# PrivEimantas/myFYP

Hardware: AMD Instinct MI355X
Metric: rounds/sec + wall-clock-to-target-acc, MNIST MLP FedAvg 8 peers at 1/2/4/8 MI355X (higher is better)
Workload: dtype fp32

## Files before the change

csrc/kernels/mlp_persistent.h:

```cpp
#pragma once
#include "mlp_fused.h"

struct MLPPersistBufs {
  bf16* h1x;
  bf16* w2x;
  bf16* dh2x;
  unsigned* flags;
  size_t flag_bytes;
  int* err;
  int plain_ok;
  int plain;
};

bool mlp_persistent_supported(const MLPArgs& a);
size_t mlp_persistent_bytes(int P, int Bpad);
size_t mlp_persistent_flag_bytes(int P);
int mlp_persistent_blocks(int P);
hipError_t mlp_persistent_prepare(const MLPArgs& a);
hipError_t mlp_launch_persistent_epoch(const MLPArgs& a, const MLPPersistBufs& pb, hipStream_t s, bool zero_flags = true);

struct MLPPersistF32Bufs {
  float* h1x;
  float* plx;
  float* dh2x;
  unsigned* gen;
  unsigned* flags;
  size_t flag_bytes;
  int* err;
  unsigned fbase;
  float* w2chk;
  int plain_ok;
  int plain;
  int plain_x;
  int c2_straight;
};

int mlp_plain_pub_mode();
bool mlp_persistent_f32_supported(const MLPArgs& a);
size_t mlp_persistent_f32_h1x_floats(int P, int Bpad);
size_t mlp_persistent_f32_bytes(int P, int Bpad);
size_t mlp_persistent_f32_flag_bytes(int P);
int mlp_persistent_f32_gang();
int mlp_persistent_f32_resident_capacity(const MLPArgs& a, int num_cus);
int mlp_persistent_f32_launch_wgs(const MLPArgs& a);
int mlp_persistent_f32_ks(const MLPArgs& a);
int mlp_persistent_f32_variant(const MLPArgs& a);
int mlp_persistent_f32_flags_per_peer();
void mlp_persistent_f32_flag_layout(int* line, int* lines_per_peer, int* full_lines);
hipError_t mlp_persistent_f32_prepare(const MLPArgs& a);
hipError_t mlp_launch_persistent_f32_epoch(const MLPArgs& a, const MLPPersistF32Bufs& pb, hipStream_t s, bool zero_flags = true,
                                           const int* active = nullptr);
void mlp_launch_eval_f32(const MLPArgs& a, int max_rows, hipStream_t s);
```

csrc/kernels/mlp_persistent_f32.hip:

```cpp
#include <atomic>

#include "mlp_persistent.h"
#include "persist_common.h"
#include "mlp_f32_common.h"

bool mlp_f32v2_supported(const MLPArgs& a);
size_t mlp_f32v2_lds(const MLPArgs& a);
size_t mlp_f32v2_bytes(int P, int Bpad);
int mlp_f32v2_launch_wgs();
int mlp_f32v2_resident_capacity(const MLPArgs& a, int num_cus);
hipError_t mlp_f32v2_prepare(const MLPArgs& a);
void mlp_f32v2_launch(const MLPArgs& a, const MLPPersistF32Bufs& pb, hipStream_t s);

#ifdef MLP_STAMPS
__device__ unsigned long long g_p32_stamps[2][128][10];
__device__ unsigned long long g_p32_epoch[4];
#define P32_STAMP(role, t, i)                                                                    \
  do {                                                                                           \
    if (p == 0 && threadIdx.x == 0 && (t) < 128) g_p32_stamps[role][t][i] = wall_clock64(); \
  } while (0)
#define P32_ESTAMP(i)                                        \
  do {                                                       \
    if (p == 0 && threadIdx.x == 0) g_p32_epoch[i] = wall_clock64(); \
  } while (0)
#define P32_STAMP_W1(t, i)                                                                   \
  do {                                                                                       \
    if (p == 0 && threadIdx.x == 64 && (t) < 128) g_p32_stamps[0][t][i] = wall_clock64(); \
  } while (0)
extern "C" int mlp_debug_persistent_f32_stamps(void* out) {
  return hipMemcpyFromSymbol(out, HIP_SYMBOL(g_p32_stamps), sizeof(g_p32_stamps)) == hipSuccess ? 0 : 1;
}
extern "C" int mlp_debug_persistent_f32_epoch_stamps(void* out) {
  return hipMemcpyFromSymbol(out, HIP_SYMBOL(g_p32_epoch), sizeof(g_p32_epoch)) == hipSuccess ? 0 : 1;
}
#else
#define P32_STAMP(role, t, i) \
  do {                        \
  } while (0)
#define P32_ESTAMP(i) \
  do {                \
  } while (0)
#define P32_STAMP_W1(t, i) \
  do {                     \
  } while (0)
#endif

__device__ int g_plain_seen[64];

namespace {

using persist::al16;
using persist::gu32;
using persist::row_max16;
using persist::row_min16;
using persist::row_sum16;
using namespace f32k;

constexpr int SMR = 2;
constexpr int LDT_PAD = 16;
constexpr int NCG = 16;
constexpr int NH = 8;
constexpr int KSMAX = 8;
constexpr int KSLAB = KSMAX + 1;
__host__ __device__ constexpr int ng_of(int KS) { return NCG * KS; }
__host__ __device__ constexpr int roles_of(int KS) { return NCG * KS + NH; }
__host__ __device__ constexpr bool xr_of(int KS, bool RH) { return KS > 1 && !RH; }
__host__ __device__ constexpr int ppl_of(int KS, bool RH = false) { return RH ? (KS == 1 ? 8 : 4) : 8 / KS; }
__host__ __device__ constexpr int grid_of(int KS, bool RH, int nr) { return RH ? ppl_of(KS, true) * nr : 8 * (NCG + NH); }
__host__ __device__ inline int kpart_begin(int ks1, int KS, int kh) { return (kh * ks1) / KS; }
constexpr int F_H1 = 0;
constexpr int F_H1P = NCG;
constexpr int F_PL = NCG + NCG * KSMAX, F_DH2 = F_PL + NH, F_DONE = F_DH2 + NH;
constexpr int FPP = F32_FPP;
constexpr int F_XCC = F32_FPP - 5;
static_assert(F_DONE + NCG * KSMAX + NH <= F_XCC, "layout-1 flags fit the shared block");
static_assert(roles_of(KSMAX) <= 5 * 32, "XCC report slots");
constexpr int F3_DH2 = NCG * KSMAX;
constexpr int F3_W2 = F3_DH2 + 4;
constexpr int F3_HP = F3_W2 + NCG;
constexpr int F3_DONE = F3_HP + 4;
static_assert(F3_DONE + NCG * KSMAX + 4 <= F_XCC, "layout-3 flags fit the shared block");
__host__ __device__ constexpr int nhr_of(int BP) { return BP / 16; }
__host__ __device__ constexpr int roles3_of(int KS, int BP) { return NCG * KS + nhr_of(BP); }
constexpr int HPW = 16 * PD2 + PD2 + 16;
__host__ __device__ inline size_t v3_extra_floats(int P) { return (size_t)P * PD2 * PD1 + (size_t)P * 2 * 4 * HPW; }
constexpr int KS1_MAX = 25;


__device__ __forceinline__ float* h1x_part(const MLPPersistF32Bufs& pb, int p, int kh, int t, int BP) {
  return pb.h1x + (((int64_t)p * KSLAB + kh) * 2 + (t & 1)) * BP * PD1;
}
__device__ __forceinline__ float* h1x_red(const MLPPersistF32Bufs& pb, int p, int t, int BP) { return h1x_part(pb, p, KSMAX, t, BP); }


__device__ __forceinline__ bf16x8 frag_b_tr_x(const bf16* base, int ld, int k0, int s, int tt, int lane) {
  const int g = lane >> 4, q = (lane & 15) >> 2, pp = lane & 3;
  const int cx = 2 * tt + (pp >> 1);
  const bf16* p0 = base + (k0 + 8 * g + q) * ld + 32 * s + (cx << 3) + 4 * (pp & 1);
  const bf16* p1 = p0 + 4 * ld;
  const mlp_s16x4 lo = __builtin_amdgcn_ds_read_tr16_b64_v4i16((mlp_lds_s16x4*)(p0));
  const mlp_s16x4 hi = __builtin_amdgcn_ds_read_tr16_b64_v4i16((mlp_lds_s16x4*)(p1));
  return __builtin_bit_cast(bf16x8, (mlp_s16x8)__builtin_shufflevector(lo, hi, 0, 1, 2, 3, 4, 5, 6, 7));
}

struct OwnerLds32 {
  int ldx;
  int ldt;
  size_t x, red, h1, dh1s, w1x, ok, total;
};
__host__ __device__ inline int kh_of(int D0, int KS) { return (ks1_of(D0) + KS - 1) / KS; }
__host__ __device__ inline OwnerLds32 owner_lds32(int Bpad, int D0, int KS) {
  OwnerLds32 L;
  L.ldx = kh_of(D0, KS) * 32 + 8;
  L.ldt = Bpad + LDT_PAD;
  const int MT = Bpad / 16;
  const size_t red = (size_t)8 * MT * 64 * 16, dh2 = (size_t)Bpad * LDD * 4;
  size_t o = 0;
  L.x = o;    o += al16((size_t)Bpad * L.ldx * 2);
  L.red = o;  o += al16(red > dh2 ? red : dh2);
  L.h1 = o;   o += al16((size_t)2 * Bpad * 16 * 4);
  L.dh1s = o; o += al16((size_t)3 * 16 * L.ldt * 2);
  L.w1x = o;  o += al16(KS == 1 ? (size_t)4 * 16 * 32 * 4 : 0);
  L.ok = o;   o += 16;
  L.total = o;
  return L;
}
struct HeadLds32 {
  size_t h1, red, h2, lg, dlog, dh2, w3, b2, b3, ok, total;
};
__host__ __device__ inline HeadLds32 head_lds32(int Bpad) {
  HeadLds32 L;
  const int MT = Bpad / 16;
  size_t o = 0;
  L.h1 = o;   o += al16((size_t)Bpad * LDH1 * 4);
  L.red = o;  o += al16((size_t)8 * MT * 64 * 16);
  L.h2 = o;   o += al16((size_t)Bpad * LD16 * 4);
  L.lg = o;   o += al16((size_t)Bpad * LD16 * 4);
  L.dlog = o; o += al16((size_t)Bpad * LD16 * 4);
  L.dh2 = o;  o += al16((size_t)Bpad * LD16 * 4);
  L.w3 = o;   o += al16((size_t)16 * LD16 * 4);
  L.b2 = o;   o += al16(4 * 16 * 4);
  L.b3 = o;   o += al16(4 * 16 * 4);
  L.ok = o;   o += 16;
  L.total = o;
  return L;
}

__host__ __device__ constexpr int rq_of(int KS) { return KS == 1 ? 3 : KS == 2 ? 2 : 1; }

template <int KS, bool RH = false, int BP = 64>
__device__ __forceinline__ bool gang_commit(const MLPArgs& a, const MLPPersistF32Bufs& pb, int p, int role, int* sOk) {
  if (pb.fbase == 0 && role == 0 && a.debug_giveup == p + 1 + 256) {
    if (threadIdx.x == 0) __hip_atomic_store(pb.err, 1, __ATOMIC_RELAXED, __HIP_MEMORY_SCOPE_AGENT);
    return false;
  }
  constexpr int FD = RH ? F3_DONE : F_DONE;
  constexpr int NR = RH ? roles3_of(KS, BP) : roles_of(KS);
  persist::publish(pb.flags, FPP, p, FD + role, pb.fbase + DONE_MARK);
  return persist::wg_wait(pb.flags, FPP, p, FD, NR, pb.fbase + DONE_MARK, pb.err, sOk);
}

template <int BP, bool ADAM, bool EXTRA, int KS, bool RH, bool FUSE = false>
__device__ void owner32(const MLPArgs& a, const MLPPersistF32Bufs& pb, int p, int g, char* smem) {
  static_assert(!FUSE || (KS == 1 && !RH && !EXTRA), "fused forward: layout 1, K split 1, no extra term");
  constexpr int MT = BP / 16;
  constexpr int RQ = rq_of(KS);
  constexpr int XPT = BP / 4;
  const int tid = threadIdx.x, lane = tid & 63;
  const int wave = __builtin_amdgcn_readfirstlane(tid >> 6);
  const int h = lane >> 4, c = lane & 15;
  const int cg = g % NCG, kh = g / NCG;
  const int D0 = a.D0;
  constexpr bool XR = xr_of(KS, RH);
  const int s0 = kpart_begin(ks1_of(D0), KS, kh);
  const int KS1 = kpart_begin(ks1_of(D0), KS, kh + 1) - s0;
  const int C0 = 32 * s0;
  const OwnerLds32 L = owner_lds32(BP, D0, KS);
  const int LDX = L.ldx, LDT = L.ldt;
  bf16* sX = reinterpret_cast<bf16*>(smem + L.x);
  f32x4* sRed = reinterpret_cast<f32x4*>(smem + L.red);
  float* sDH2 = reinterpret_cast<float*>(smem + L.red);
  float* sH1 = reinterpret_cast<float*>(smem + L.h1);
  bf16* sD3 = reinterpret_cast<bf16*>(smem + L.dh1s);
  float* sW1x = reinterpret_cast<float*>(smem + L.w1x);
  int* sOk = reinterpret_cast<int*>(smem + L.ok);
  const OptParams& o = a.opt;
  const int4 ctl = a.ctl[p];
  const bool fresh = (ctl.x & 2) != 0;
  const int n = ctl.y;
  const int nsteps = (n + a.B - 1) / a.B;
  const int64_t pS = (int64_t)p * a.S;
  const float wdmu = o.weight_decay + (a.anchor != nullptr ? o.mu : 0.f);

  float w1[RQ][8], m1[RQ][8], v1[RQ][8], e1[RQ][8];
  const int orow = NCG * cg + c;
#pragma unroll
  for (int q = 0; q < RQ + 1; ++q) {
    const int s = wave + 8 * q;
    if (q == RQ && (KS != 1 || s >= KS1)) break;
#pragma unroll
    for (int half = 0; half < 2; ++half) {
      const int k = C0 + 32 * s + 16 * half + 4 * h;
      float4 wv = {0.f, 0.f, 0.f, 0.f}, mv = wv, vv = wv, ev = wv;
      if (s < KS1 && k < D0) {
        const int64_t idx = pS + a.off_w1 + (int64_t)orow * D0 + k;
        wv = *reinterpret_cast<const float4*>(a.params + idx);
        if (!fresh) {
          mv = *reinterpret_cast<const float4*>(a.m + idx);
          if (ADAM) vv = *reinterpret_cast<const float4*>(a.v + idx);
        }
        if (EXTRA) ev = float4{extra_at(a, idx), extra_at(a, idx + 1), extra_at(a, idx + 2), extra_at(a, idx + 3)};
      } else if (s < KS1 && k == D0) {
        const int64_t idx = pS + a.off_b1 + orow;
        wv.x = a.params[idx];
        if (!fresh) {
          mv.x = a.m[idx];
          if (ADAM) vv.x = a.v[idx];
        }
        if (EXTRA) ev.x = extra_at(a, idx);
      }
      if (q < RQ) {
        const float wa[4] = {wv.x, wv.y, wv.z, wv.w}, ma[4] = {mv.x, mv.y, mv.z, mv.w}, va[4] = {vv.x, vv.y, vv.z, vv.w},
                    ea[4] = {ev.x, ev.y, ev.z, ev.w};
#pragma unroll
        for (int i = 0; i < 4; ++i) {
          w1[q][4 * half + i] = wa[i];
          m1[q][4 * half + i] = ma[i];
          v1[q][4 * half + i] = va[i];
          e1[q][4 * half + i] = ea[i];
        }
      } else {
        const int off = c * 32 + 16 * half + 4 * h;
        *reinterpret_cast<float4*>(sW1x + off) = wv;
        *reinterpret_cast<float4*>(sW1x + 512 + off) = mv;
        *reinterpret_cast<float4*>(sW1x + 1024 + off) = vv;
        *reinterpret_cast<float4*>(sW1x + 1536 + off) = ev;
      }
    }
  }
  float w2c[4], m2c[4], v2c[4], e2c[4];
#pragma unroll
  for (int i = 0; i < 4; ++i) {
    const int64_t idx = pS + a.off_w2 + (int64_t)(16 * wave + 4 * h + i) * PD1 + NCG * cg + c;
    w2c[i] = a.params[idx];
    m2c[i] = fresh ? 0.f : a.m[idx];
    v2c[i] = (ADAM && !fresh) ? a.v[idx] : 0.f;
    e2c[i] = EXTRA ? extra_at(a, idx) : 0.f;
  }

  auto bias_chunk = [](bool valid) { return uint4{valid ? 0x3F80u : 0u, 0u, 0u, 0u}; };
  auto xw_stage = [&](int t, int lv) {
    const int rows = rows_at(a, n, t);
#pragma unroll
    for (int k = 0; k < XPT; ++k) {
      const int q = k / (BP / 16), kk = k % (BP / 16);
      if (q > RQ || (q == RQ && KS != 1)) break;
      const int s = wave + 8 * q;
      const int idx = kk * 64 + lv;
      const int r = idx >> 2, col = 32 * s + 8 * (idx & 3), gcol = C0 + col;
      if (s < KS1 && gcol < D0) {
        const bf16* src = a.Xb16 + ((int64_t)p * a.xb_rows + (int64_t)t * a.B + r) * D0 + gcol;
        *reinterpret_cast<uint4*>(sX + r * LDX + col) = r < rows ? *reinterpret_cast<const uint4*>(src) : uint4{0u, 0u, 0u, 0u};
      } else if (s < KS1 && gcol == D0) {
        *reinterpret_cast<uint4*>(sX + r * LDX + col) = bias_chunk(r < rows);
      }
    }
  };
  {
// ... 36 lines not shown
      bf16x8 af[MT];
#pragma unroll
      for (int mt = 0; mt < MT; ++mt) {
        const bf16* xp = sX + (16 * mt + cq) * LDX + 32 * s + 4 * (hq & 1);
        af[mt] = cat8(*reinterpret_cast<const bf16x4*>(xp + ((hq >> 1) << 3)), *reinterpret_cast<const bf16x4*>(xp + ((2 + (hq >> 1)) << 3)));
      }
#pragma unroll
      for (int mt = 0; mt < MT; ++mt) acc[mt] = mfma_bf16(af[mt], bl, acc[mt]);
#pragma unroll
      for (int mt = 0; mt < MT; ++mt) acc[mt] = mfma_bf16(af[mt], bm, acc[mt]);
#pragma unroll
      for (int mt = 0; mt < MT; ++mt) acc[mt] = mfma_bf16(af[mt], bh, acc[mt]);
      return;
    }
#pragma unroll
    for (int mt = 0; mt < MT; ++mt) {
      const bf16* xp = sX + (16 * mt + cq) * LDX + 32 * s + 4 * (hq & 1);
      const bf16x8 af = cat8(*reinterpret_cast<const bf16x4*>(xp + ((hq >> 1) << 3)), *reinterpret_cast<const bf16x4*>(xp + ((2 + (hq >> 1)) << 3)));
      acc[mt] = mfma3(af, bh, bm, bl, acc[mt]);
    }
  };
  auto fwd_all = [&](f32x4(&acc)[MT]) {
#pragma unroll
    for (int mt = 0; mt < MT; ++mt) acc[mt] = zero4();
#pragma unroll
    for (int q = 0; q < (KS == 1 ? RQ + 1 : RQ); ++q) {
      fwd_kstep(q, acc);
      __builtin_amdgcn_sched_barrier(0);
    }
  };
  auto h1_publish = [&](int t, const f32x4(&acc)[MT]) -> bool {
    const int rows = rows_at(a, n, t);
    float* sH1c = sH1 + (t & 1) * BP * 16;
    int tq = tid;
    asm volatile("" : "+v"(tq));
#pragma unroll
    for (int mt = 0; mt < MT; ++mt) sRed[(wave * MT + mt) * 64 + (tq & 63)] = acc[mt];
    lds_barrier();
    if (tq < MT * 64) {
      const int mt = tq >> 6, hh = (tq & 63) >> 4, cc = tq & 15;
      f32x4 s = sRed[mt * 64 + (tq & 63)];
#pragma unroll
      for (int w = 1; w < 8; ++w) s += sRed[(w * MT + mt) * 64 + (tq & 63)];
#pragma unroll
      for (int i = 0; i < 4; ++i) {
        const int b = 16 * mt + 4 * hh + i;
        const float v = b < rows ? (KS == 1 ? fmaxf(s[i], 0.f) : s[i]) : 0.f;
        sH1c[b * 16 + cc] = v;
        persist::pub32(pb.plain, h1x_part(pb, p, kh, t, BP) + (unsigned)(b * PD1 + NCG * cg + cc), v);
      }
    }
    if (g == 0) P32_STAMP(0, t, 1);
    persist::publish_p(pb.flags, FPP, p, XR ? F_H1P + cg * KS + kh : F_H1 + g, pb.fbase + (unsigned)(t + 1), pb.plain);
    if (XR) {
      if (!persist::wg_wait(pb.flags, FPP, p, F_H1P + cg * KS, KS, pb.fbase + (unsigned)(t + 1), pb.err, sOk)) return false;
      if (tid < BP * 4) {
        const int b = tid >> 2, c4 = 4 * (tid & 3);
        float4 u[KS];
#pragma unroll
        for (int k2 = 0; k2 < KS; ++k2)
          u[k2] = k2 == kh ? *reinterpret_cast<const float4*>(sH1c + b * 16 + c4)
                           : ld_sc1_16(rsrc_of(h1x_part(pb, p, k2, t, BP), BP * PD1 * 4), (b * PD1 + NCG * cg + c4) * 4);
        float4 sum = u[0];
#pragma unroll
        for (int k2 = 1; k2 < KS; ++k2) {
          sum.x += u[k2].x;
          sum.y += u[k2].y;
          sum.z += u[k2].z;
          sum.w += u[k2].w;
        }
        const float4 r = {fmaxf(sum.x, 0.f), fmaxf(sum.y, 0.f), fmaxf(sum.z, 0.f), fmaxf(sum.w, 0.f)};
        *reinterpret_cast<float4*>(sH1c + b * 16 + c4) = r;
        if (kh == 0) persist::pub128(pb.plain_x, h1x_red(pb, p, t, BP), BP * PD1 * 4, (b * PD1 + NCG * cg + c4) * 4, __builtin_bit_cast(u32x4, r));
      }
      if (kh == 0)
        persist::publish_p(pb.flags, FPP, p, F_H1 + cg, pb.fbase + (unsigned)(t + 1), pb.plain_x);
      else
        __syncthreads();
    }
    if (g == 0) P32_STAMP(0, t, 2);
    return true;
  };
  if (tid == 0) sOk[1] = 1;
  __syncthreads();

  if (FUSE && nsteps > 0) {
    f32x4 acc[MT];
    fwd_all(acc);
    if (!h1_publish(0, acc)) return;
  }

  persist::BiasCorr bc;
  bc.init(o, ctl.z);
  float lr_t = 0.f, inv_bc2 = 0.f;
  constexpr bool SI = KS == 1 && !RH && !EXTRA;
  const bool straight = SI && pb.c2_straight != 0 && wave + 8 * (RQ - 1) < KS1;
#pragma unroll
  for (int body = 0; body < (SI ? 2 : 1); ++body) {
  const bool ST = SI && body == 1;
  if (SI && straight != ST) continue;
  for (int t = 0; t < nsteps; ++t) {
    int tv = tid;
    asm volatile("" : "+v"(tv));
    const float lr_prev = lr_t, inv_prev = inv_bc2;
    const unsigned t1 = (unsigned)(t + 1);
    bc.next(o, lr_t, inv_bc2);
    float* sH1c = sH1 + (t & 1) * BP * 16;
    if (g == 0) P32_STAMP(0, t, 0);

    if constexpr (!FUSE) {
      f32x4 acc[MT];
      fwd_all(acc);
      if (g == 0) P32_STAMP(0, t, 7);
      if (!h1_publish(t, acc)) return;
    }

    if (!RH && t > 0) w2_replica_update(t - 1, lr_prev, inv_prev);
    if (g == 0) P32_STAMP(0, t, 3);

    const bool more = t + 1 < nsteps;
    if (more) {
      const int rows_n = rows_at(a, n, t + 1);
      unsigned sink = 0;
      int xi = lane;
      if (FUSE) asm volatile("" : "+v"(xi));
      const bf16* xbase = a.Xb16 + ((int64_t)p * a.xb_rows + (int64_t)(t + 1) * a.B) * D0;
      const bf16* xrow = xbase + (unsigned)(xi * D0);
#pragma unroll
      for (int q = 0; q < (KS == 1 ? RQ + 1 : RQ); ++q) {
        const int s = wave + 8 * q;
        const int r = lane;
        if (s < KS1 && C0 + 32 * s < D0 && r < rows_n && r < BP)
          sink ^= *reinterpret_cast<const unsigned*>(xrow + C0 + 32 * s);
      }
      asm volatile("" ::"v"(sink));
    }

    constexpr int XQF = FUSE ? BP / 16 : 1;
    uint4 xqf[XQF];
    const __amdgpu_buffer_rsrc_t r_xn =
        rsrc_of(a.Xb16 + ((int64_t)p * a.xb_rows + (int64_t)(t + 1) * a.B) * D0, more ? rows_at(a, n, t + 1) * D0 * 2 : 0);
    auto xq_load = [&](int q, bool chk = true) __attribute__((always_inline)) {
      const int s = wave + 8 * q;
      if (chk && s >= KS1) return;
      int lx = lane;
      if (chk)
        asm volatile("" : "+v"(lx));
      else
        lx = tv & 63;
#pragma unroll
      for (int kk = 0; kk < XQF; ++kk) {
        const int idx = kk * 64 + lx;
        const int r = idx >> 2, gcol = C0 + 32 * s + 8 * (idx & 3);
        unsigned off = (unsigned)(r * D0 + gcol) * 2u;
        asm("" : "+v"(off));
        off = gcol < D0 ? off : 0x7FFFFFF0u;
        asm("" : "+v"(off));
        xqf[kk] = __builtin_bit_cast(uint4, __builtin_amdgcn_raw_buffer_load_b128(r_xn, off, 0, 0));
      }
    };
    if constexpr (FUSE) xq_load(0);

    const float* dh2_t = pb.dh2x + ((int64_t)p * 2 + (t & 1)) * BP * PD2 * 2;
    const __amdgpu_buffer_rsrc_t r_dh2 = rsrc_of(dh2_t, BP * PD2 * 8);
    if (!persist::wg_wait(pb.flags, FPP, p, RH ? F3_DH2 : F_DH2, RH ? nhr_of(BP) : NH, pb.fbase + t1, pb.err, sOk)) return;
    if (g == 0) P32_STAMP(0, t, 4);
    if (KS > 1 && !XR) {
      if (tid < BP * 4) {
        const int b = tid >> 2, c4 = 4 * (tid & 3);
        float4 sum = {0.f, 0.f, 0.f, 0.f};
#pragma unroll
        for (int k2 = 0; k2 < KS; ++k2) {
          float4 v;
          if (k2 == kh) {
            v = *reinterpret_cast<const float4*>(sH1c + b * 16 + c4);
          } else {
            const __amdgpu_buffer_rsrc_t r = rsrc_of(h1x_part(pb, p, k2, t, BP), BP * PD1 * 4);
            v = ld_sc1_16(r, (b * PD1 + NCG * cg + c4) * 4);
          }
          sum.x += v.x;
          sum.y += v.y;
          sum.z += v.z;
          sum.w += v.w;
        }
        *reinterpret_cast<float4*>(sH1c + b * 16 + c4) = float4{fmaxf(sum.x, 0.f), fmaxf(sum.y, 0.f), fmaxf(sum.z, 0.f), fmaxf(sum.w, 0.f)};
      }
    }
    {
      float4 v[BP / 16];
#pragma unroll
      for (int k = 0; k < BP / 16; ++k) v[k] = ld_sc1_16(r_dh2, (tv + NT * k) * 16);
#pragma unroll
      for (int k = 0; k < BP / 16; ++k) {
        const int e = tv + NT * k;
        *reinterpret_cast<float4*>(sDH2 + (e >> 5) * LDD + 4 * (e & 31)) = v[k];
      }
    }
    lds_barrier();
    if (sOk[1] == 0) return;
    {
      f32x4 acc1[MT];
#pragma unroll
      for (int mt = 0; mt < MT; ++mt) {
        const float4 av = *reinterpret_cast<const float4*>(sDH2 + (16 * mt + c) * LDD + 16 * wave + 4 * h);
        f32x4 acc = mfma_f32(av.x, w2c[0], zero4());
        acc = mfma_f32(av.y, w2c[1], acc);
        acc = mfma_f32(av.z, w2c[2], acc);
        acc1[mt] = mfma_f32(av.w, w2c[3], acc);
      }
      f32x4 dw2 = zero4();
      if (RH) {
        const float* h1p = sH1c;
#pragma unroll
        for (int kb = 0; kb < BP / 4; ++kb) dw2 = mfma_f32(sDH2[(4 * kb + h) * LDD + 16 * wave + c], h1p[(4 * kb + h) * 16 + c], dw2);
      }
      lds_barrier();
#pragma unroll
      for (int mt = 0; mt < MT; ++mt) sRed[(wave * MT + mt) * 64 + lane] = acc1[mt];
      if (RH) {
#pragma unroll
        for (int i = 0; i < 4; ++i) upd32<ADAM, EXTRA>(o, dw2[i], w2c[i], m2c[i], v2c[i], e2c[i], lr_t, inv_bc2, wdmu);
        if (kh == 0) {
          float* w2x = pb.dh2x + (int64_t)a.P * 2 * BP * PD2 * 2 + (int64_t)p * PD2 * PD1;
#pragma unroll
          for (int i = 0; i < 4; ++i) persist::pub32(pb.plain, w2x + (16 * wave + 4 * h + i) * PD1 + NCG * cg + c, w2c[i]);
        }
      }
    }
    if (RH && kh == 0) {
      persist::publish_p(pb.flags, FPP, p, F3_W2 + cg, pb.fbase + (unsigned)(t + 2), pb.plain);
    } else {
      lds_barrier();
    }
    if (tv < MT * 64) {
      const int mt = tv >> 6, hh = (tv & 63) >> 4, cc = tv & 15;
      f32x4 s = sRed[mt * 64 + (tv & 63)];
#pragma unroll
      for (int w = 1; w < 8; ++w) s += sRed[(w * MT + mt) * 64 + (tv & 63)];
      bf16x4 dh, dm, dl;
#pragma unroll
      for (int i = 0; i < 4; ++i) {
        const float d = sH1c[(16 * mt + 4 * hh + i) * 16 + cc] > 0.f ? s[i] : 0.f;
        const bf16 x0 = (bf16)d;
        const float r = d - (float)x0;
        const bf16 x1 = (bf16)r;
        dh[i] = x0;
        dm[i] = x1;
        dl[i] = (bf16)(r - (float)x1);
      }
      const int off = cc * LDT + 16 * mt + 4 * hh;
      *reinterpret_cast<bf16x4*>(sD3 + off) = dh;
      *reinterpret_cast<bf16x4*>(sD3 + 16 * LDT + off) = dm;
      *reinterpret_cast<bf16x4*>(sD3 + 32 * LDT + off) = dl;
    }
    lds_barrier();
    if (g == 0) P32_STAMP(0, t, 5);
    {
      int lv = lane;
      asm volatile("" : "+v"(lv));
      f32x4 accF[FUSE ? MT : 1];
#pragma unroll
      for (int mt = 0; mt < (FUSE ? MT : 1); ++mt) accF[mt] = zero4();
      const int rows_next = more ? rows_at(a, n, t + 1) : 0;
      const bf16* xnext = a.Xb16 + ((int64_t)p * a.xb_rows + (int64_t)(t + 1) * a.B) * D0;
#pragma unroll
      for (int q = 0; q < (KS == 1 ? RQ + 1 : RQ); ++q) {
        const bool STq = ST && q < RQ;
        const int s = wave + 8 * q;
        if (STq || s < KS1) {
          int lq = lane;
          asm volatile("" : "+v"(lq));
          const bf16* dfrag = sD3 + (lq & 15) * LDT + 8 * (lq >> 4);
          constexpr int XQ = BP / 16;
          uint4 xq[XQ];
#pragma unroll
          for (int kk = 0; kk < XQ; ++kk) {
            if constexpr (FUSE) {
              xq[kk] = xqf[FUSE ? kk : 0];
              continue;
            }
            const int idx = kk * 64 + lv;
            const int r = idx >> 2, col = 32 * s + 8 * (idx & 3), gcol = C0 + col;
            if (STq) {
              unsigned off = (unsigned)(r * D0 + gcol) * 2u;
              asm("" : "+v"(off));
              off = gcol < D0 ? off : 0x7FFFFFF0u;
              asm("" : "+v"(off));
              xq[kk] = __builtin_bit_cast(uint4, __builtin_amdgcn_raw_buffer_load_b128(r_xn, off, 0, 0));
              continue;
            }
            const bool xl = more && gcol < D0 && r < rows_next;
            xq[kk] = xl ? *reinterpret_cast<const uint4*>(xnext + (unsigned)(r * D0 + gcol)) : uint4{0u, 0u, 0u, 0u};
          }
#pragma unroll
          for (int tt = 0; tt < 2; ++tt) {
            f32x4 acc = zero4();
#pragma unroll
            for (int kb = 0; kb < BP / 32; ++kb)
              acc = mfma3(frag_b_tr_x(sX, LDX, 32 * kb, s, tt, lq), ld8(dfrag + 32 * kb), ld8(dfrag + 16 * LDT + 32 * kb),
                          ld8(dfrag + 32 * LDT + 32 * kb), acc);
            if (q < RQ) {
              const int qq = q < RQ ? q : 0;
#pragma unroll
              for (int i = 0; i < 4; ++i)
                upd32<ADAM, EXTRA>(o, acc[i], w1[qq][4 * tt + i], m1[qq][4 * tt + i], v1[qq][4 * tt + i], e1[qq][4 * tt + i], lr_t, inv_bc2, wdmu);
            } else {
              const int off = (lq & 15) * 32 + 16 * tt + 4 * (lq >> 4);
              float4 w = *reinterpret_cast<float4*>(sW1x + off), m = *reinterpret_cast<float4*>(sW1x + 512 + off),
                     v = *reinterpret_cast<float4*>(sW1x + 1024 + off), e = *reinterpret_cast<float4*>(sW1x + 1536 + off);
              upd32<ADAM, EXTRA>(o, acc[0], w.x, m.x, v.x, e.x, lr_t, inv_bc2, wdmu);
              upd32<ADAM, EXTRA>(o, acc[1], w.y, m.y, v.y, e.y, lr_t, inv_bc2, wdmu);
              upd32<ADAM, EXTRA>(o, acc[2], w.z, m.z, v.z, e.z, lr_t, inv_bc2, wdmu);
              upd32<ADAM, EXTRA>(o, acc[3], w.w, m.w, v.w, e.w, lr_t, inv_bc2, wdmu);
              *reinterpret_cast<float4*>(sW1x + off) = w;
              *reinterpret_cast<float4*>(sW1x + 512 + off) = m;
              *reinterpret_cast<float4*>(sW1x + 1024 + off) = v;
            }
          }
          if (STq || more) {
#pragma unroll
            for (int kk = 0; kk < XQ; ++kk) {
              const int idx = kk * 64 + lv;
              const int r = idx >> 2, col = 32 * s + 8 * (idx & 3), gcol = C0 + col;
              if (STq || (SI && q == RQ)) {
                const unsigned b1 = (gcol == D0 && r < rows_next) ? 0x3F80u : 0u;
                *reinterpret_cast<u32x4*>(sX + r * LDX + col) = u32x4{xq[kk].x | b1, xq[kk].y, xq[kk].z, xq[kk].w};
              } else if (gcol < D0) {
                *reinterpret_cast<uint4*>(sX + r * LDX + col) = xq[kk];
              } else if (gcol == D0) {
                *reinterpret_cast<uint4*>(sX + r * LDX + col) = bias_chunk(r < rows_next);
              }
            }
          }
        }
        if constexpr (FUSE) {
          if (q + 1 < (KS == 1 ? RQ + 1 : RQ)) xq_load(q + 1, !STq);
          if (STq)
            fwd_kstep(q, accF, false);
          else if (more)
            fwd_kstep(q, accF);
        }
      }
      if constexpr (FUSE) {
        if (g == 0) P32_STAMP(0, t, 6);
        if (g == 0) P32_STAMP_W1(t, 8);
        if (more) {
          if (!h1_publish(t + 1, accF)) return;
        } else {
          __syncthreads();
        }
      }
    }
    if constexpr (!FUSE) {
      __syncthreads();
      if (g == 0) P32_STAMP(0, t, 6);
    }
    }
  }

  if (!gang_commit<KS, RH, BP>(a, pb, p, g, sOk)) return;
  if (g == 0) P32_ESTAMP(2);
  int lw = lane;
  int64_t pS_w = pS;
  asm volatile("" : "+v"(lw), "+s"(pS_w));
  const int hw = lw >> 4, cw = lw & 15;
  const int orow_w = NCG * cg + cw;
#pragma unroll
  for (int q = 0; q < (KS == 1 ? RQ + 1 : RQ); ++q) {
    const int s = wave + 8 * q;
#pragma unroll
    for (int half = 0; half < 2; ++half) {
      const int k = C0 + 32 * s + 16 * half + 4 * hw;
      if (s >= KS1 || k > D0) continue;
      float4 w, m, v;
      if (q < RQ) {
        const int qq = q < RQ ? q : 0;
        const int j0 = 4 * half;
        w = float4{w1[qq][j0], w1[qq][j0 + 1], w1[qq][j0 + 2], w1[qq][j0 + 3]};
        m = float4{m1[qq][j0], m1[qq][j0 + 1], m1[qq][j0 + 2], m1[qq][j0 + 3]};
        v = float4{v1[qq][j0], v1[qq][j0 + 1], v1[qq][j0 + 2], v1[qq][j0 + 3]};
      } else {
        const int off = cw * 32 + 16 * half + 4 * hw;
        w = *reinterpret_cast<float4*>(sW1x + off);
        m = *reinterpret_cast<float4*>(sW1x + 512 + off);
        v = *reinterpret_cast<float4*>(sW1x + 1024 + off);
      }
      if (k < D0) {
        const int64_t idx = pS_w + a.off_w1 + (int64_t)orow_w * D0 + k;
        *reinterpret_cast<float4*>(a.params + idx) = w;
        *reinterpret_cast<float4*>(a.m + idx) = m;
        if (ADAM) *reinterpret_cast<float4*>(a.v + idx) = v;
      } else {
        const int64_t idx = pS_w + a.off_b1 + orow_w;
        a.params[idx] = w.x;
        a.m[idx] = m.x;
        if (ADAM) a.v[idx] = v.x;
      }
    }
  }
  if (RH && kh == 0) {
#pragma unroll
    for (int i = 0; i < 4; ++i) {
      const int64_t idx = pS_w + a.off_w2 + (int64_t)(16 * wave + 4 * hw + i) * PD1 + NCG * cg + cw;
      a.params[idx] = w2c[i];
      a.m[idx] = m2c[i];
      if (ADAM) a.v[idx] = v2c[i];
    }
  }
  if (!RH && pb.w2chk != nullptr) {
    if (nsteps > 0) w2_replica_update(nsteps - 1, lr_t, inv_bc2);
#pragma unroll
    for (int i = 0; i < 4; ++i) pb.w2chk[(int64_t)p * PD2 * PD1 + (int64_t)(16 * wave + 4 * hw + i) * PD1 + NCG * cg + cw] = w2c[i];
  }
}

template <int BP, bool ADAM, bool EXTRA, int KS>
__device__ void head32(const MLPArgs& a, const MLPPersistF32Bufs& pb, int p, int hd, char* smem) {
  constexpr int MT = BP / 16;
  constexpr bool XR = xr_of(KS, false);
  const int tid = threadIdx.x, lane = tid & 63;
  const int wave = __builtin_amdgcn_readfirstlane(tid >> 6);
  const int h = lane >> 4, c = lane & 15;
  const int D3 = a.D3;
  const HeadLds32 L = head_lds32(BP);
  float* sH1 = reinterpret_cast<float*>(smem + L.h1);
  f32x4* sRed = reinterpret_cast<f32x4*>(smem + L.red);
  float* sH2 = reinterpret_cast<float*>(smem + L.h2);
  float* sLg = reinterpret_cast<float*>(smem + L.lg);
// ... 995 lines not shown
  return v == 2 ? mlp_f32v2_launch_wgs() : grid_of(f32_ks(a), v == 3, roles_for(a, f32_ks(a)));
}
int mlp_persistent_f32_resident_capacity(const MLPArgs& a, int num_cus) {
  const int v = f32_variant(a);
  return v == 2 ? mlp_f32v2_resident_capacity(a, num_cus) : resident_capacity_ks(a, num_cus, f32_ks(a), v == 3);
}
int mlp_persistent_f32_flags_per_peer() { return FPP * persist::FLAG_LINE; }
void mlp_persistent_f32_flag_layout(int* line, int* lines_per_peer, int* full_lines) {
  *line = persist::FLAG_LINE;
  *lines_per_peer = FPP;
  *full_lines = FPP - F_XCC;
}

hipError_t mlp_persistent_f32_prepare(const MLPArgs& a) {
  hipError_t e;
  for (int KS = 1; KS <= KSMAX; KS *= 2) {
    const int lds = (int)persistent_f32_lds_ks(a, KS);
    if (KS > 2) {
      if (a.Bpad != 64) continue;
      e = KS == 4 ? prepare_f32_bp<64, 4>(lds) : prepare_f32_bp<64, 8>(lds);
      if (e != hipSuccess) return e;
      continue;
    }
    e = KS == 1 ? (a.Bpad == 64 ? prepare_f32_bp<64, 1>(lds) : prepare_f32_bp<32, 1>(lds))
                : (a.Bpad == 64 ? prepare_f32_bp<64, 2>(lds) : prepare_f32_bp<32, 2>(lds));
    if (e != hipSuccess) return e;
    if (v3_supported(a)) {
      const int l3 = (int)persistent_f32_lds_ks(a, KS, true);
      e = KS == 1 ? (a.Bpad == 64 ? prepare_f32_bp<64, 1, true>(l3) : prepare_f32_bp<32, 1, true>(l3))
                  : (a.Bpad == 64 ? prepare_f32_bp<64, 2, true>(l3) : prepare_f32_bp<32, 2, true>(l3));
      if (e != hipSuccess) return e;
    }
  }
  if (mlp_f32v2_supported(a)) {
    e = mlp_f32v2_prepare(a);
    if (e != hipSuccess) return e;
  }
  return hipFuncSetAttribute((const void*)mlp_eval_f32, hipFuncAttributeMaxDynamicSharedMemorySize, (int)eval_lds32(a.D0));
}

static std::atomic<int> g_plain_override{-1};
int mlp_plain_pub_mode() {
  const int o = g_plain_override.load(std::memory_order_relaxed);
  if (o >= 0) return o;
  static const int v = [] {
    const char* e = getenv("MYFYP_F32_PLAIN_PUB");
    return e != nullptr ? atoi(e) : 1;
  }();
  return v;
}
extern "C" int mlp_set_plain_pub(int mode) { return g_plain_override.exchange(mode < 0 ? -1 : mode); }
extern "C" int mlp_debug_plain_seen(int* out) {
  return hipMemcpyFromSymbol(out, HIP_SYMBOL(g_plain_seen), sizeof(g_plain_seen)) == hipSuccess ? 0 : 1;
}

static std::atomic<int> g_fuse_override{-1};
static std::atomic<int> g_fuse_last{-1};
static int f32_fwd_fuse_mode() {
  const int o = g_fuse_override.load(std::memory_order_relaxed);
  if (o >= 0) return o;
  static const int v = [] {
    const char* e = getenv("MYFYP_F32_FWD_FUSE");
    return e != nullptr ? atoi(e) : 1;
  }();
  return v;
}
extern "C" int mlp_set_f32_fwd_fuse(int mode) { return g_fuse_override.exchange(mode < 0 ? -1 : mode); }
extern "C" int mlp_f32_fwd_fuse_last() { return g_fuse_last.load(std::memory_order_relaxed); }

static std::atomic<int> g_straight_override{-1};
static std::atomic<int> g_straight_last{-1};
static int f32_c2_straight_mode() {
  const int o = g_straight_override.load(std::memory_order_relaxed);
  if (o >= 0) return o;
  static const int v = [] {
    const char* e = getenv("MYFYP_F32_C2_STRAIGHT");
    return e != nullptr ? atoi(e) : 1;
  }();
  return v;
}
extern "C" int mlp_set_f32_c2_straight(int mode) { return g_straight_override.exchange(mode < 0 ? -1 : mode); }
extern "C" int mlp_f32_c2_straight_last() { return g_straight_last.load(std::memory_order_relaxed); }

hipError_t mlp_launch_persistent_f32_epoch(const MLPArgs& a, const MLPPersistF32Bufs& pb_in, hipStream_t s, bool zero_flags, const int* active) {
  MLPPersistF32Bufs pb = pb_in;
  pb.plain_ok = mlp_plain_pub_mode();
  pb.plain = 0;
  if (zero_flags) {
    hipError_t e = hipMemsetAsync(pb.flags, 0, pb.flag_bytes, s);
    if (e != hipSuccess) return e;
  }
  if (f32_variant(a) == 2) {
    mlp_f32v2_launch(a, pb, s);
    return hipGetLastError();
  }
  const int KS = f32_ks(a);
  const bool rh = f32_variant(a) == 3;
  const int ppl = ppl_of(KS, rh);
  const size_t lds = persistent_f32_lds_ks(a, KS, rh);
  const bool fuse = f32_fwd_fuse_mode() != 0 && fuse_inst(KS, rh) && a.anchor == nullptr && a.cg == nullptr;
  g_fuse_last.store(fuse ? 1 : 0, std::memory_order_relaxed);
  pb.c2_straight = f32_c2_straight_mode() != 0 ? 1 : 0;
  g_straight_last.store(pb.c2_straight && !rh && KS == 1 && 7 + 8 * (rq_of(1) - 1) < ks1_of(a.D0) ? 1 : 0, std::memory_order_relaxed);
  auto group_live = [&](int p0) {
    if (active == nullptr) return true;
    for (int p = p0; p < p0 + ppl && p < a.P; ++p)
      if (active[p]) return true;
    return false;
  };
  for (int attempt = 0; attempt < 2; ++attempt)
    for (int p0 = 0; p0 < a.P; p0 += ppl) {
      if (!group_live(p0)) continue;
      if (rh) {
        if (KS == 2) {
          if (a.Bpad == 64) launch_f32_bp<64, 2, true>(a, pb, s, p0, lds, attempt, fuse);
          else launch_f32_bp<32, 2, true>(a, pb, s, p0, lds, attempt, fuse);
        } else {
          if (a.Bpad == 64) launch_f32_bp<64, 1, true>(a, pb, s, p0, lds, attempt, fuse);
          else launch_f32_bp<32, 1, true>(a, pb, s, p0, lds, attempt, fuse);
        }
      } else if (KS == 8) {
        launch_f32_bp<64, 8>(a, pb, s, p0, lds, attempt, fuse);
      } else if (KS == 4) {
        launch_f32_bp<64, 4>(a, pb, s, p0, lds, attempt, fuse);
      } else if (KS == 2) {
        if (a.Bpad == 64) launch_f32_bp<64, 2>(a, pb, s, p0, lds, attempt, fuse);
        else launch_f32_bp<32, 2>(a, pb, s, p0, lds, attempt, fuse);
      } else {
        if (a.Bpad == 64) launch_f32_bp<64, 1>(a, pb, s, p0, lds, attempt, fuse);
        else launch_f32_bp<32, 1>(a, pb, s, p0, lds, attempt, fuse);
      }
    }
  return hipGetLastError();
}

static int eval_wgs_cap() {
  static const int v = [] {
    const char* e = getenv("MYFYP_EVAL_WGS");
    return e != nullptr ? atoi(e) : 32;
  }();
  return v;
}
void mlp_launch_eval_f32(const MLPArgs& a, int max_rows, hipStream_t s) {
  if (max_rows <= 0) return;
  const int chunks = (max_rows + EV_ROWS - 1) / EV_ROWS, cap = eval_wgs_cap();
  const int per_peer = cap > 0 ? (cap / a.P > 0 ? cap / a.P : 1) : chunks;
  const dim3 grid(chunks < per_peer ? chunks : per_peer, a.P);
  hipLaunchKernelGGL(mlp_eval_f32, grid, dim3(NT), eval_lds32(a.D0), s, a);
}

extern "C" int myfyp_warm_mlp_f32() {
  hipFuncAttributes attr;
  return hipFuncGetAttributes(&attr, reinterpret_cast<const void*>(&mlp_eval_f32)) == hipSuccess ? 0 : 1;
}
```

myfyp_amd/ops/_native.py:

```python

from __future__ import annotations

import ctypes
import os
import threading
from typing import Optional

_LIB: Optional[ctypes.CDLL] = None
_FAST: Optional[ctypes.PyDLL] = None
_LOCK = threading.Lock()
_ERR: Optional[str] = None

LIB_DIR = os.path.join(os.path.dirname(os.path.dirname(os.path.abspath(__file__))), "_native")
LIB_PATH = os.environ.get("MYFYP_NATIVE_LIB") or os.path.join(LIB_DIR, "libmyfyp_hip.so")

c_void_p = ctypes.c_void_p
c_int = ctypes.c_int
c_int64 = ctypes.c_int64
c_float = ctypes.c_float

_SIGNATURES = {
    "myfyp_version": (c_int, []),
    "myfyp_last_error": (ctypes.c_char_p, []),
    "myfyp_weighted_sum": (c_int, [c_void_p, c_void_p, c_void_p, c_int, c_int64, c_void_p]),
    "myfyp_stacked_weighted_sum": (c_int, [c_void_p, c_void_p, c_int, c_int64, c_int64, c_void_p, c_float, c_void_p]),
    "myfyp_broadcast_rows": (c_int, [c_void_p, c_void_p, c_int, c_int64, c_int64, c_void_p, c_void_p]),
    "myfyp_coordinate_median": (c_int, [c_void_p, c_void_p, c_int, c_int64, c_void_p]),
    "myfyp_coordinate_median_multi": (c_int, [c_void_p, c_int, c_void_p, c_int, c_int64, c_void_p]),
    "myfyp_trimmed_mean_multi": (c_int, [c_void_p, c_int, c_void_p, c_int, c_int, c_int64, c_void_p]),
    "myfyp_krum_grid": (c_int, [c_int64, c_int]),
    "myfyp_krum_multi": (c_int, [c_void_p, c_int, c_void_p, c_void_p, c_int, c_int, c_int, c_int64, c_void_p, c_void_p, c_void_p, c_void_p, c_void_p]),
    "myfyp_scaffold_reduce": (c_int, [c_void_p, c_void_p, c_void_p, c_void_p, c_int, c_int64, c_void_p]),
    "myfyp_scaffold_apply": (c_int, [c_void_p, c_int, c_void_p, c_void_p, c_void_p, c_int, c_float, c_int64, c_void_p]),
    "myfyp_adam_step": (
        c_int,
        [c_void_p, c_void_p, c_void_p, c_void_p, c_void_p, c_int64, c_float, c_float, c_float, c_float, c_float, c_int, c_void_p, c_void_p, c_void_p, c_float, c_void_p],
    ),
    "myfyp_sgd_step": (c_int, [c_void_p, c_void_p, c_void_p, c_int64, c_float, c_float, c_float, c_int, c_void_p, c_void_p, c_void_p, c_float, c_void_p]),
    "myfyp_scale_add_noise": (c_int, [c_void_p, c_int64, c_float, c_float, ctypes.c_uint64, c_void_p]),

    "mlp_shape_ok": (c_int, [c_int, c_int, c_int, c_int]),
    "mlp_engine_create": (c_void_p, [c_int, c_int, c_int, c_int, c_int, c_int]),
    "mlp_engine_destroy": (None, [c_void_p]),
    "mlp_engine_numel": (c_int64, [c_void_p]),
    "mlp_engine_bind_params": (c_int, [c_void_p, c_void_p, c_void_p, c_void_p, c_void_p, c_void_p, c_int64]),
    "mlp_engine_set_train_data": (c_int, [c_void_p, c_void_p, c_void_p, c_void_p, c_void_p, c_int64, c_int]),
    "mlp_engine_set_test_data": (c_int, [c_void_p, c_void_p, c_void_p, c_void_p, c_int]),
    "mlp_engine_set_counts": (c_int, [c_void_p, c_void_p, c_void_p]),
    "mlp_engine_set_optimizer": (c_int, [c_void_p, c_int, c_float, c_float, c_float, c_float, c_float, c_float, c_int, c_float]),
    "mlp_engine_set_extras": (c_int, [c_void_p, c_void_p, c_void_p, c_void_p]),
    "mlp_engine_begin": (c_int, [c_void_p, c_void_p, c_void_p]),
    "mlp_engine_run_epoch": (c_int, [c_void_p, c_void_p, c_void_p]),
    "mlp_engine_run_epoch_pub": (c_int, [c_void_p, c_void_p, c_int, c_void_p]),
    "mlp_engine_drain_prep": (c_int, [c_void_p]),
    "mlp_engine_run_epoch_eager": (c_int, [c_void_p, c_void_p, c_void_p]),
    "mlp_engine_read_stats": (c_int, [c_void_p, c_void_p, c_void_p, c_void_p]),
    "mlp_engine_eval": (c_int, [c_void_p, c_void_p, c_void_p, c_void_p, c_void_p, c_void_p]),
    "mlp_engine_stats_async": (c_int, [c_void_p, c_int, c_void_p]),
    "mlp_engine_eval_async": (c_int, [c_void_p, c_void_p, c_int, c_void_p]),
    "mlp_engine_fetch": (c_int, [c_void_p, c_int, c_void_p, c_void_p, c_void_p]),
    "mlp_engine_ring_size": (c_int, []),
    "mlp_engine_set_persistent": (c_int, [c_void_p, c_int]),
    "mlp_engine_zero_state": (c_int, [c_void_p, c_void_p]),
    "mlp_engine_set_shuffle": (c_int, [c_void_p, c_int]),
    "mlp_engine_set_epoch_seed": (c_int, [c_void_p, ctypes.c_uint64]),
    "mlp_engine_set_next_epoch_seed": (c_int, [c_void_p, ctypes.c_uint64]),
    "myfyp_fedavg_stacked_reduce": (c_int, [c_void_p, c_void_p, c_int, c_int64, c_int64, c_void_p, c_void_p]),
    "myfyp_fedavg_stacked_apply": (c_int, [c_void_p, c_void_p, c_int, c_int64, c_int64, c_void_p, c_void_p]),
    "myfyp_fedavg_stacked_local": (c_int, [c_void_p, c_int, c_int64, c_int64, c_void_p, c_void_p, c_void_p]),
    "myfyp_fedavg_bucket_reduce": (c_int, [c_void_p, c_void_p, c_void_p, c_int, c_int64, c_int64, c_void_p, c_void_p]),
    "myfyp_fedavg_bucket_apply": (c_int, [c_void_p, c_void_p, c_void_p, c_int, c_int64, c_int64, c_void_p, c_void_p]),
    "myfyp_fedavg_bucket_reduce2": (c_int, [c_void_p, c_void_p, c_void_p, c_void_p, c_void_p, c_int, c_int64, c_int64, c_void_p, c_void_p]),
    "myfyp_fedavg_delayed_land": (c_int, [c_void_p, c_void_p, c_int64, c_void_p, c_void_p, c_int, c_int64, c_int64, c_void_p, c_void_p]),
    "myfyp_neighbor_mix_stacked": (c_int, [c_void_p, c_int, c_int64, c_int64, c_void_p, c_void_p]),
    "mlp_engine_uses_persistent": (c_int, [c_void_p]),
    "mlp_engine_set_precision": (c_int, [c_void_p, c_int]),
    "mlp_f32_ok": (c_int, [c_int, c_int, c_int, c_int, c_int]),
    "mlp_engine_set_w2chk": (c_int, [c_void_p, c_void_p]),
    "mlp_engine_recoveries": (c_int, [c_void_p]),
    "mlp_engine_graph_launch_stats": (c_int, [c_void_p, c_void_p]),
    "mlp_engine_set_f32_ks": (c_int, [c_void_p, c_int]),
    "mlp_engine_set_reserved_cus": (c_int, [c_void_p, c_int]),
    "mlp_engine_f32_ks": (c_int, [c_void_p]),
    "mlp_engine_set_f32_variant": (c_int, [c_void_p, c_int]),
    "mlp_engine_f32_variant": (c_int, [c_void_p]),
    "mlp_engine_debug_giveup": (c_int, [c_void_p, c_int, c_int]),
    "mlp_engine_debug_poison_flags": (c_int, [c_void_p, c_int]),
    "mlp_engine_prepare": (c_int, [c_void_p, c_void_p]),
    "myfyp_warm_all": (c_int, [c_int]),
    "mlp_set_plain_pub": (c_int, [c_int]),
    "mlp_debug_plain_seen": (c_int, [c_void_p]),
    "mlp_set_f32_fwd_fuse": (c_int, [c_int]),
    "mlp_f32_fwd_fuse_last": (c_int, []),
    "mlp_set_f32_c2_straight": (c_int, [c_int]),
    "mlp_f32_c2_straight_last": (c_int, []),
    "mlp_debug_stamps": (c_int, [c_void_p]),
    "mlp_debug_persistent_f32_stamps": (c_int, [c_void_p]),
}


def load(required: bool = False) -> Optional[ctypes.CDLL]:
    global _LIB, _ERR
    if _LIB is not None:
        return _LIB
    with _LOCK:
        if _LIB is None and _ERR is None:
            if not os.path.exists(LIB_PATH):
                _ERR = f"native library not built: {LIB_PATH} (run python -m myfyp_amd.ops.build)"
            else:
                try:
                    lib = ctypes.CDLL(LIB_PATH, mode=ctypes.RTLD_GLOBAL)
                    for name, (res, args) in _SIGNATURES.items():
                        fn = getattr(lib, name, None)
                        if fn is None:
                            continue
                        fn.restype = res
                        fn.argtypes = args
                    _LIB = lib
                except OSError as e:
                    _ERR = f"failed to load {LIB_PATH}: {e}"
    if _LIB is None and required:
        raise RuntimeError(_ERR or "native library unavailable")
    return _LIB


def load_fast() -> ctypes.PyDLL:
    global _FAST
    if _FAST is not None:
        return _FAST
    load(required=True)
    with _LOCK:
        if _FAST is None:
            lib = ctypes.PyDLL(LIB_PATH, mode=ctypes.RTLD_GLOBAL)
            for name, (res, args) in _SIGNATURES.items():
                fn = getattr(lib, name, None)
                if fn is None:
                    continue
                fn.restype = res
                fn.argtypes = args
            _FAST = lib
    return _FAST


def debug_update_scale() -> float:
    v = os.environ.get("MYFYP_DEBUG_LR_SCALE")
    return float(v) if v else 1.0


_WARM: set = set()


def warm_device(index: int, family: str = "mlp") -> None:
    key = (index, family)
    if key in _WARM:
        return
    lib = load(required=True)
    fn = getattr(lib, "myfyp_warm_all", None)
    if fn is not None:
        bad = int(fn(1 if family == "mlp" else 2))
        if bad:
            raise RuntimeError(f"native code objects: {bad} kernel unit(s) failed to load on device {index}")
    _WARM.add(key)


def available() -> bool:
    return load() is not None


def error() -> Optional[str]:
    load()
    return _ERR


def check(rc: int, what: str) -> None:
    if rc != 0:
        msg = _LIB.myfyp_last_error().decode() if _LIB is not None else "?"
        raise RuntimeError(f"{what} failed (rc={rc}): {msg}")
```

Baseline: 706.0.

## Split the last K step's W1 tile updates onto two helper waves

```diff
diff --git a/csrc/kernels/mlp_persistent.h b/csrc/kernels/mlp_persistent.h
--- a/csrc/kernels/mlp_persistent.h
+++ b/csrc/kernels/mlp_persistent.h
@@ -33,6 +33,7 @@
   int plain;
   int plain_x;
   int c2_straight;
+  int k24_split;
 };
 
 int mlp_plain_pub_mode();
diff --git a/csrc/kernels/mlp_persistent_f32.hip b/csrc/kernels/mlp_persistent_f32.hip
--- a/csrc/kernels/mlp_persistent_f32.hip
+++ b/csrc/kernels/mlp_persistent_f32.hip
@@ -27,6 +27,10 @@
   do {                                                                                       \
     if (p == 0 && threadIdx.x == 64 && (t) < 128) g_p32_stamps[0][t][i] = wall_clock64(); \
   } while (0)
+#define P32_STAMP_WV(t, i, w)                                                                      \
+  do {                                                                                             \
+    if (p == 0 && threadIdx.x == 64 * (w) && (t) < 128) g_p32_stamps[0][t][i] = wall_clock64(); \
+  } while (0)
 extern "C" int mlp_debug_persistent_f32_stamps(void* out) {
   return hipMemcpyFromSymbol(out, HIP_SYMBOL(g_p32_stamps), sizeof(g_p32_stamps)) == hipSuccess ? 0 : 1;
 }
@@ -43,6 +47,9 @@
 #define P32_STAMP_W1(t, i) \
   do {                     \
   } while (0)
+#define P32_STAMP_WV(t, i, w) \
+  do {                        \
+  } while (0)
 #endif
 
 __device__ int g_plain_seen[64];
@@ -58,6 +65,14 @@
 
 constexpr int SMR = 2;
 constexpr int LDT_PAD = 16;
+#ifndef K24_WA
+#define K24_WA 1
+#endif
+#ifndef K24_WB
+#define K24_WB 2
+#endif
+static_assert(K24_WA > 0 && K24_WA < 8 && K24_WB > 0 && K24_WB < 8 && K24_WA != K24_WB, "K step 24's helpers: two waves other than wave 0");
+typedef __attribute__((address_space(3))) unsigned lds_u32;
 constexpr int NCG = 16;
 constexpr int NH = 8;
 constexpr int KSMAX = 8;
@@ -106,7 +121,7 @@
 struct OwnerLds32 {
   int ldx;
   int ldt;
-  size_t x, red, h1, dh1s, w1x, ok, total;
+  size_t x, red, h1, dh1s, w1x, ok, k24, total;
 };
 __host__ __device__ inline int kh_of(int D0, int KS) { return (ks1_of(D0) + KS - 1) / KS; }
 __host__ __device__ inline OwnerLds32 owner_lds32(int Bpad, int D0, int KS) {
@@ -122,6 +137,7 @@
   L.dh1s = o; o += al16((size_t)3 * 16 * L.ldt * 2);
   L.w1x = o;  o += al16(KS == 1 ? (size_t)4 * 16 * 32 * 4 : 0);
   L.ok = o;   o += 16;
+  L.k24 = o;  o += 16;
   L.total = o;
   return L;
 }
@@ -184,6 +200,7 @@
   bf16* sD3 = reinterpret_cast<bf16*>(smem + L.dh1s);
   float* sW1x = reinterpret_cast<float*>(smem + L.w1x);
   int* sOk = reinterpret_cast<int*>(smem + L.ok);
+  lds_u32* sK24 = (lds_u32*)(smem + L.k24);
   const OptParams& o = a.opt;
   const int4 ctl = a.ctl[p];
   const bool fresh = (ctl.x & 2) != 0;
@@ -386,6 +403,7 @@
     return true;
   };
   if (tid == 0) sOk[1] = 1;
+  if (tid < 2) sK24[tid] = 0u;
   __syncthreads();
 
   if (FUSE && nsteps > 0) {
@@ -399,10 +417,52 @@
   float lr_t = 0.f, inv_bc2 = 0.f;
   constexpr bool SI = KS == 1 && !RH && !EXTRA;
   const bool straight = SI && pb.c2_straight != 0 && wave + 8 * (RQ - 1) < KS1;
-#pragma unroll
-  for (int body = 0; body < (SI ? 2 : 1); ++body) {
-  const bool ST = SI && body == 1;
-  if (SI && straight != ST) continue;
+  const bool split = straight && pb.k24_split != 0 && KS1 == KS1_MAX;
+  constexpr int S24 = 8 * RQ;
+  auto k24_tile = [&](int tt, unsigned t1) __attribute__((always_inline)) {
+    int lq = lane;
+    asm volatile("" : "+v"(lq));
+    const bf16* dfrag = sD3 + (lq & 15) * LDT + 8 * (lq >> 4);
+    f32x4 acc = zero4();
+#pragma unroll
+    for (int kb = 0; kb < BP / 32; ++kb)
+      acc = mfma3(frag_b_tr_x(sX, LDX, 32 * kb, S24, tt, lq), ld8(dfrag + 32 * kb), ld8(dfrag + 16 * LDT + 32 * kb),
+                  ld8(dfrag + 32 * LDT + 32 * kb), acc);
+    const int off = (lq & 15) * 32 + 16 * tt + 4 * (lq >> 4);
+    float4 w = *reinterpret_cast<float4*>(sW1x + off), m = *reinterpret_cast<float4*>(sW1x + 512 + off),
+           v = *reinterpret_cast<float4*>(sW1x + 1024 + off), e = *reinterpret_cast<float4*>(sW1x + 1536 + off);
+    upd32<ADAM, EXTRA>(o, acc[0], w.x, m.x, v.x, e.x, lr_t, inv_bc2, wdmu);
+    upd32<ADAM, EXTRA>(o, acc[1], w.y, m.y, v.y, e.y, lr_t, inv_bc2, wdmu);
+    upd32<ADAM, EXTRA>(o, acc[2], w.z, m.z, v.z, e.z, lr_t, inv_bc2, wdmu);
+    upd32<ADAM, EXTRA>(o, acc[3], w.w, m.w, v.w, e.w, lr_t, inv_bc2, wdmu);
+    *reinterpret_cast<float4*>(sW1x + off) = w;
+    *reinterpret_cast<float4*>(sW1x + 512 + off) = m;
+    *reinterpret_cast<float4*>(sW1x + 1024 + off) = v;
+    __hip_atomic_store(sK24 + tt, t1, __ATOMIC_RELEASE, __HIP_MEMORY_SCOPE_WORKGROUP);
+  };
+  auto k24_wait = [&](unsigned t1) __attribute__((always_inline)) {
+    unsigned long long t0 = 0;
+    for (unsigned it = 1;; ++it) {
+      const unsigned v0 = __hip_atomic_load(sK24, __ATOMIC_ACQUIRE, __HIP_MEMORY_SCOPE_WORKGROUP);
+      const unsigned v1 = __hip_atomic_load(sK24 + 1, __ATOMIC_ACQUIRE, __HIP_MEMORY_SCOPE_WORKGROUP);
+      if (__all(v0 >= t1 && v1 >= t1)) break;
+      if (persist::poll_check(it)) {
+        if (__builtin_amdgcn_readfirstlane(__hip_atomic_load((gu32*)pb.err, __ATOMIC_RELAXED, __HIP_MEMORY_SCOPE_AGENT)) != 0u) break;
+        const unsigned long long now = wall_clock64();
+        if (t0 == 0) t0 = now;
+        if (now - t0 > persist::SPIN_TICKS) {
+          if (lane == 0) __hip_atomic_store((gu32*)pb.err, 1u, __ATOMIC_RELAXED, __HIP_MEMORY_SCOPE_AGENT);
+          break;
+        }
+      }
+      persist::poll_sleep();
+    }
+  };
+#pragma unroll
+  for (int body = 0; body < (SI ? 3 : 1); ++body) {
+  const bool ST = SI && body >= 1;
+  const bool SP = SI && body == 2;
+  if (SI && (straight ? (split ? 2 : 1) : 0) != body) continue;
   for (int t = 0; t < nsteps; ++t) {
     int tv = tid;
     asm volatile("" : "+v"(tv));
@@ -567,6 +627,7 @@
       for (int mt = 0; mt < (FUSE ? MT : 1); ++mt) accF[mt] = zero4();
       const int rows_next = more ? rows_at(a, n, t + 1) : 0;
       const bf16* xnext = a.Xb16 + ((int64_t)p * a.xb_rows + (int64_t)(t + 1) * a.B) * D0;
+      if (SP && (wave == K24_WA || wave == K24_WB)) k24_tile(wave == K24_WB ? 1 : 0, t1);
 #pragma unroll
       for (int q = 0; q < (KS == 1 ? RQ + 1 : RQ); ++q) {
         const bool STq = ST && q < RQ;
@@ -596,8 +657,9 @@
             const bool xl = more && gcol < D0 && r < rows_next;
             xq[kk] = xl ? *reinterpret_cast<const uint4*>(xnext + (unsigned)(r * D0 + gcol)) : uint4{0u, 0u, 0u, 0u};
           }
-#pragma unroll
-          for (int tt = 0; tt < 2; ++tt) {
+          if (SP && q == RQ) k24_wait(t1);
+#pragma unroll
+          for (int tt = 0; tt < (SP && q == RQ ? 0 : 2); ++tt) {
             f32x4 acc = zero4();
 #pragma unroll
             for (int kb = 0; kb < BP / 32; ++kb)
@@ -648,6 +710,7 @@
       if constexpr (FUSE) {
         if (g == 0) P32_STAMP(0, t, 6);
         if (g == 0) P32_STAMP_W1(t, 8);
+        if (g == 0) P32_STAMP_WV(t, 9, K24_WA);
         if (more) {
           if (!h1_publish(t + 1, accF)) return;
         } else {
@@ -1809,6 +1872,20 @@
 extern "C" int mlp_set_f32_c2_straight(int mode) { return g_straight_override.exchange(mode < 0 ? -1 : mode); }
 extern "C" int mlp_f32_c2_straight_last() { return g_straight_last.load(std::memory_order_relaxed); }
 
+static std::atomic<int> g_k24_override{-1};
+static std::atomic<int> g_k24_last{-1};
+static int f32_k24_split_mode() {
+  const int o = g_k24_override.load(std::memory_order_relaxed);
+  if (o >= 0) return o;
+  static const int v = [] {
+    const char* e = getenv("MYFYP_F32_K24_SPLIT");
+    return e != nullptr ? atoi(e) : 1;
+  }();
+  return v;
+}
+extern "C" int mlp_set_f32_k24_split(int mode) { return g_k24_override.exchange(mode < 0 ? -1 : mode); }
+extern "C" int mlp_f32_k24_split_last() { return g_k24_last.load(std::memory_order_relaxed); }
+
 hipError_t mlp_launch_persistent_f32_epoch(const MLPArgs& a, const MLPPersistF32Bufs& pb_in, hipStream_t s, bool zero_flags, const int* active) {
   MLPPersistF32Bufs pb = pb_in;
   pb.plain_ok = mlp_plain_pub_mode();
@@ -1829,6 +1906,8 @@
   g_fuse_last.store(fuse ? 1 : 0, std::memory_order_relaxed);
   pb.c2_straight = f32_c2_straight_mode() != 0 ? 1 : 0;
   g_straight_last.store(pb.c2_straight && !rh && KS == 1 && 7 + 8 * (rq_of(1) - 1) < ks1_of(a.D0) ? 1 : 0, std::memory_order_relaxed);
+  pb.k24_split = f32_k24_split_mode() != 0 ? 1 : 0;
+  g_k24_last.store(pb.k24_split && pb.c2_straight && !rh && KS == 1 && ks1_of(a.D0) == KS1_MAX ? 1 : 0, std::memory_order_relaxed);
   auto group_live = [&](int p0) {
     if (active == nullptr) return true;
     for (int p = p0; p < p0 + ppl && p < a.P; ++p)
diff --git a/myfyp_amd/ops/_native.py b/myfyp_amd/ops/_native.py
--- a/myfyp_amd/ops/_native.py
+++ b/myfyp_amd/ops/_native.py
@@ -94,6 +94,8 @@
     "mlp_f32_fwd_fuse_last": (c_int, []),
     "mlp_set_f32_c2_straight": (c_int, [c_int]),
     "mlp_f32_c2_straight_last": (c_int, []),
+    "mlp_set_f32_k24_split": (c_int, [c_int]),
+    "mlp_f32_k24_split_last": (c_int, []),
     "mlp_debug_stamps": (c_int, [c_void_p]),
     "mlp_debug_persistent_f32_stamps": (c_int, [c_void_p]),
 }
```

New measurement: 715.4, median of 6. 1.3% higher.
